# RDG0818/MAZero

Measured on NVIDIA B200. Metric: mcts_sims_per_sec, higher is better.
Workload: dtype bf16

## Files before the change

mazero_b200/csrc/infer_hmma.cuh:

```cuda
#pragma once
#include <cuda_bf16.h>

#include "../../include/maz_infer.h"
#include "umma.cuh"

namespace maz {
namespace hmma {

using namespace umma;

constexpr int H = 128, NHEAD = 8, HD = 16, GH = 64, PH = 32, SUP = 11, NLAYER = 3;
constexpr int NCHUNK = MAZ_INFER_NCHUNK, NSLOT = 3;
constexpr int TM = 32;
#ifndef MAZ_HMMA_NQ
#define MAZ_HMMA_NQ 4
#endif
constexpr int NQ = MAZ_HMMA_NQ;
constexpr int NT = H / NQ / 8;
constexpr int GT = GH / NQ / 8;
constexpr int CW = H / NQ, FW = GH / NQ;
static_assert(NQ == 4 || NQ == 8, "NQ");
constexpr int NCONS = 64 * NQ, NTHREADS = NCONS + 32;
constexpr int PAD = 8;
constexpr int LDA = (H + PAD) * 2;
// ... 117 lines not shown
#pragma unroll GEMM_UNROLL
    for (int ks = 0; ks < KS; ++ks) {
        const int cur = ks & 1, nxt = cur ^ 1;
        if (ks + 1 < KS) {
            ldsm4(aa + 32u * (ks + 1), a[nxt]);
#pragma unroll
            for (int p = 0; p < NT / 2; ++p) ldsm4(wa + (uint32_t)(16 * p) * ldw + 32u * (ks + 1), b[nxt][p]);
        }
#pragma unroll
        for (int p = 0; p < NT / 2; ++p) {
            mma16816(acc[2 * p], a[cur], b[cur][p][0], b[cur][p][1]);
            mma16816(acc[2 * p + 1], a[cur], b[cur][p][2], b[cur][p][3]);
        }
    }
}
template <int NT>
__device__ __forceinline__ void gemm_rt(float (&acc)[NT][4], const Thr &th, uint32_t a_tile, int lda, uint32_t w_slot, int ldw, int n0, int K)
{
    const uint32_t aa = th.a_addr(a_tile, lda), wa = th.w_addr(w_slot, ldw, n0);
#pragma unroll 1
    for (int k0 = 0; k0 < K; k0 += 16) {
        uint32_t a[4], b[NT / 2][4];
        ldsm4(aa + 2u * k0, a);
#pragma unroll
        for (int p = 0; p < NT / 2; ++p) ldsm4(wa + (uint32_t)(16 * p) * ldw + 2u * k0, b[p]);
#pragma unroll
        for (int p = 0; p < NT / 2; ++p) {
            mma16816(acc[2 * p], a, b[p][0], b[p][1]);
            mma16816(acc[2 * p + 1], a, b[p][2], b[p][3]);
        }
    }
}

__device__ __forceinline__ void issue_chunk(const Desc &d, int k, int slot, uint64_t *bar_full)
{
    HSM_DECL;
    const uint32_t nbytes = (d.dbg_flags & 4) ? 16u : d.chunk_bytes[k];
    const uint8_t *src = reinterpret_cast<const uint8_t *>(d.wpk) + d.chunk_off[k];
    uint8_t *dst = hsm + OFF_W + (size_t)slot * SLOT_BYTES;
    mbar_expect_tx(&bar_full[slot], nbytes);
    for (uint32_t o = 0; o < nbytes; o += PIECE) {
        const uint32_t n = (nbytes - o < PIECE) ? (nbytes - o) : PIECE;
        bulk_g2s(dst + o, src + o, n, &bar_full[slot]);
    }
}

struct Ring {
    uint64_t *full, *empty;
    int c;
    __device__ __forceinline__ uint32_t acquire(int ahead = 0)
    {
        const int cc = c + ahead, s = cc % NSLOT;
        mbar_wait(&full[s], (cc / NSLOT) & 1);
        return sbase() + OFF_W + (uint32_t)s * SLOT_BYTES;
    }
    __device__ __forceinline__ void release(int lane, int n = 1)
    {
        __syncwarp();
        if (lane == 0)
            for (int i = 0; i < n; ++i) mbar_arrive(&empty[(c + i) % NSLOT]);
        c += n;
    }
};

__device__ __forceinline__ void cta_sync() { named_bar_sync(1, NCONS); }

template <int NT>
__device__ __forceinline__ void zero(float (&acc)[NT][4])
{
#pragma unroll
    for (int i = 0; i < NT; ++i) acc[i][0] = acc[i][1] = acc[i][2] = acc[i][3] = 0.f;
}
template <int NT>
__device__ __forceinline__ void copy(float (&dst)[NT][4], const float (&src)[NT][4])
{
#pragma unroll
    for (int i = 0; i < NT; ++i) { dst[i][0] = src[i][0]; dst[i][1] = src[i][1]; dst[i][2] = src[i][2]; dst[i][3] = src[i][3]; }
}

template <int NT>
__device__ __forceinline__ void add_bias(float (&acc)[NT][4], const Thr &th, uint32_t b, int n0)
{
#pragma unroll
    for (int nt = 0; nt < NT; ++nt) {
        const float2 v = ldp2(b + 4u * (n0 + 8 * nt + 2 * th.t));
        acc[nt][0] += v.x; acc[nt][1] += v.y; acc[nt][2] += v.x; acc[nt][3] += v.y;
    }
}
template <int NT>
__device__ __forceinline__ void store_tile(uint32_t tile, int ld, const Thr &th, int n0, const float (&acc)[NT][4])
{
#pragma unroll
    for (int nt = 0; nt < NT; ++nt) {
        const int c = n0 + 8 * nt + 2 * th.t;
        sts32(tile + (uint32_t)th.rA * ld + 2u * c, pack2(acc[nt][0], acc[nt][1]));
        sts32(tile + (uint32_t)th.rB * ld + 2u * c, pack2(acc[nt][2], acc[nt][3]));
    }
}
// ... 8 lines not shown
}

template <int NT>
__device__ __forceinline__ void stats_write(const float (&v)[NT][4], const Thr &th, uint32_t stat)
{
    float s0 = 0.f, q0 = 0.f, s1 = 0.f, q1 = 0.f;
#pragma unroll
    for (int nt = 0; nt < NT; ++nt) {
        s0 += v[nt][0] + v[nt][1]; q0 += v[nt][0] * v[nt][0] + v[nt][1] * v[nt][1];
        s1 += v[nt][2] + v[nt][3]; q1 += v[nt][2] * v[nt][2] + v[nt][3] * v[nt][3];
    }
#pragma unroll
    for (int o = 1; o <= 2; o <<= 1) {
        s0 += __shfl_xor_sync(0xffffffffu, s0, o); q0 += __shfl_xor_sync(0xffffffffu, q0, o);
        s1 += __shfl_xor_sync(0xffffffffu, s1, o); q1 += __shfl_xor_sync(0xffffffffu, q1, o);
    }
    if (th.t == 0) {
        sts2f(stat + (uint32_t)(th.rA * NQ + th.nq) * 8u, s0, q0);
        sts2f(stat + (uint32_t)(th.rB * NQ + th.nq) * 8u, s1, q1);
    }
}
__device__ __forceinline__ void stats_read(uint32_t stat, int row, float inv_width, float &mean, float &rstd)
{
    float4 v[NQ / 2];
#pragma unroll
    for (int i = 0; i < NQ / 2; ++i) v[i] = lds4v(stat + (uint32_t)row * (NQ * 8u) + 16u * i);
    float s = 0.f, q = 0.f;
#pragma unroll
    for (int i = 0; i < NQ / 2; ++i) { s += v[i].x + v[i].z; q += v[i].y + v[i].w; }
    mean = s * inv_width;
    rstd = rsqrtf(fmaxf(q * inv_width - mean * mean, 0.f) + 1e-5f);
}

__device__ __forceinline__ void layer_norm128(float (&x)[NT][4], const Thr &th, uint32_t gam, uint32_t bet, int n0, bool relu_after)
{
    const uint32_t stat = sbase() + OFF_STAT;
    stats_write<NT>(x, th, stat);
    cta_sync();
    float mA, sA, mB, sB;
    stats_read(stat, th.rA, 1.f / H, mA, sA);
    stats_read(stat, th.rB, 1.f / H, mB, sB);
#pragma unroll
    for (int nt = 0; nt < NT; ++nt) {
        const int c = n0 + 8 * nt + 2 * th.t;
        const float2 gg = ldp2(gam + 4u * c), bb = ldp2(bet + 4u * c);
        x[nt][0] = (x[nt][0] - mA) * sA * gg.x + bb.x; x[nt][1] = (x[nt][1] - mA) * sA * gg.y + bb.y;
        x[nt][2] = (x[nt][2] - mB) * sB * gg.x + bb.x; x[nt][3] = (x[nt][3] - mB) * sB * gg.y + bb.y;
    }
    if (relu_after) relu<NT>(x);
}

__device__ __forceinline__ RowInfo row_info(int r)
{
    uint32_t a, b, c, e;
    lds4u(sbase() + OFF_ROW + 16u * r, a, b, c, e);
    RowInfo ri;
    ri.root = (int)a; ri.agent = (int)b; ri.valid = (int)c; ri.r0 = (int)e;
    return ri;
}

static __device__ __noinline__ void stage_gather(const Desc &d, const SimIo io)
{
    HSM_DECL;
    const int tid = threadIdx.x, r = tid >> 3, part = tid & 7;
    if (tid >= TM * 8) return;
    const RowInfo ri = row_info(r);
    uint32_t w[8] = {0, 0, 0, 0, 0, 0, 0, 0};
    int action = -1;
    if (ri.valid) {
        const int ix = io.idx_x ? __ldcg(io.idx_x + ri.root) : 0;
        if (d.greedy_pool == nullptr || d.cur < 0)
            action = __ldcg(io.actions + (size_t)ri.root * d.N + ri.agent);
        else if (ri.agent == d.cur)
            action = __ldcg(io.actions + ri.root);
        else if (ri.agent < d.cur)
            action = d.factor ? __ldcg(d.factor + (size_t)ri.root * d.N + ri.agent) : 0;
        else
            action = __ldcg(d.greedy_pool + ((size_t)ix * d.B + ri.root) * d.N + ri.agent);
        const float *h = d.pool + ((size_t)ix * d.B + ri.root) * (size_t)(d.N * H) + (size_t)ri.agent * H + part * 16;
#pragma unroll
        for (int i = 0; i < 4; ++i) {
            const float4 v = __ldcg(reinterpret_cast<const float4 *>(h) + i);
            w[2 * i] = pack2(v.x, v.y);
            w[2 * i + 1] = pack2(v.z, v.w);
        }
    }
    uint4 *dst = reinterpret_cast<uint4 *>(hsm + OFF_HH + (size_t)r * LDA + part * 32);
    dst[0] = make_uint4(w[0], w[1], w[2], w[3]);
    dst[1] = make_uint4(w[4], w[5], w[6], w[7]);
    if (part * 8 < d.KA) {
        const int c0 = part * 8;
        uint32_t o[4];
#pragma unroll
        for (int i = 0; i < 4; ++i) o[i] = pack2((c0 + 2 * i == action) ? 1.f : 0.f, (c0 + 2 * i + 1 == action) ? 1.f : 0.f);
        *reinterpret_cast<uint4 *>(hsm + OFF_ONE + (size_t)r * LDO + c0 * 2) = make_uint4(o[0], o[1], o[2], o[3]);
    }
}

static __device__ __noinline__ void stage_inproj(const Desc &d, Ring &ring, float (&xio)[NT][4])
{
    const Thr th;
    const uint32_t sb = sbase();
    const int n0 = CW * th.nq, ldo = (d.KA + PAD) * 2;
    float x[NT][4];
    zero<NT>(x);
    uint32_t w = ring.acquire();
    gemm_fixed<NT, 8>(x, th, sb + OFF_HH, LDA, w, LDA, n0);
    ring.release(th.lane);
    w = ring.acquire();
    gemm_rt<NT>(x, th, sb + OFF_ONE, LDO, w, ldo, n0, d.KA);
    ring.release(th.lane);
    add_bias<NT>(x, th, sb + OFF_P + 4u * d.o_bin, n0);
    const uint32_t pA = sb + OFF_P + 4u * (d.o_pos + row_info(th.rA).agent * H), pB = sb + OFF_P + 4u * (d.o_pos + row_info(th.rB).agent * H);
#pragma unroll
    for (int nt = 0; nt < NT; ++nt) {
        const int c = n0 + 8 * nt + 2 * th.t;
        const float2 a = ldp2(pA + 4u * c), b = ldp2(pB + 4u * c);
        x[nt][0] = fmaxf(x[nt][0], 0.f) + a.x; x[nt][1] = fmaxf(x[nt][1], 0.f) + a.y;
        x[nt][2] = fmaxf(x[nt][2], 0.f) + b.x; x[nt][3] = fmaxf(x[nt][3], 0.f) + b.y;
    }
    store_tile<NT>(sb + OFF_X, LDA, th, n0, x);
    copy<NT>(xio, x);
    cta_sync();
}

static __device__ __noinline__ void stage_qkv(Ring &ring, uint32_t lv)
{
    const Thr th;
    const uint32_t sb = sbase();
    const int n0 = CW * th.nq;
    float acc[3 * NT][4];
    zero<3 * NT>(acc);
    uint32_t wa[3];
#pragma unroll
    for (int i = 0; i < 3; ++i) wa[i] = th.w_addr(ring.acquire(i), LDA, n0);
    const uint32_t aa = th.a_addr(sb + OFF_X, LDA);
    constexpr int PW = NT / 2, NP = 3 * PW;
    uint32_t a[2][4], b[2][NP][4];
    ldsm4(aa, a[0]);
#pragma unroll
    for (int p = 0; p < NP; ++p) ldsm4(wa[p / PW] + (uint32_t)(16 * (p % PW)) * LDA, b[0][p]);
#pragma unroll GEMM_UNROLL
    for (int ks = 0; ks < 8; ++ks) {
        const int cur = ks & 1, nxt = cur ^ 1;
        if (ks + 1 < 8) {
            ldsm4(aa + 32u * (ks + 1), a[nxt]);
#pragma unroll
            for (int p = 0; p < NP; ++p) ldsm4(wa[p / PW] + (uint32_t)(16 * (p % PW)) * LDA + 32u * (ks + 1), b[nxt][p]);
        }
#pragma unroll
        for (int p = 0; p < NP; ++p) {
            mma16816(acc[2 * p], a[cur], b[cur][p][0], b[cur][p][1]);
            mma16816(acc[2 * p + 1], a[cur], b[cur][p][2], b[cur][p][3]);
        }
    }
    ring.release(th.lane, 3);
#pragma unroll
    for (int which = 0; which < 3; ++which) {
#pragma unroll
        for (int nt = 0; nt < NT; ++nt) {
            const int c = n0 + 8 * nt + 2 * th.t;
            const float2 bv = ldp2(lv + 4u * (which * H + c));
            const float *v = acc[which * NT + nt];
            sts32(sb + OFF_Q + (uint32_t)th.rA * LDQ + 2u * (which * H + c), pack2(v[0] + bv.x, v[1] + bv.y));
            sts32(sb + OFF_Q + (uint32_t)th.rB * LDQ + 2u * (which * H + c), pack2(v[2] + bv.x, v[3] + bv.y));
        }
    }
    cta_sync();
}

__device__ __forceinline__ void unpack16(const uint32_t (&w)[8], float (&f)[16])
{
#pragma unroll
    for (int i = 0; i < 8; ++i) {
        f[2 * i] = __uint_as_float(w[i] << 16);
        f[2 * i + 1] = __uint_as_float(w[i] & 0xffff0000u);
    }
}
__device__ __forceinline__ void lds32B(uint32_t saddr, uint32_t (&w)[8])
{
    lds4u(saddr, w[0], w[1], w[2], w[3]);
    lds4u(saddr + 16u, w[4], w[5], w[6], w[7]);
}

template <int NN>
__device__ __forceinline__ void attention_small(uint32_t qbase, int r0, int hh, const float (&q)[16], float (&o)[16])
{
    float s[NN];
    uint32_t kw[NN][8], vw[NN][8];
#pragma unroll
    for (int j = 0; j < NN; ++j) {
        const uint32_t kr = qbase + (uint32_t)(r0 + j) * LDQ + H * 2 + hh * 32;
        lds32B(kr, kw[j]);
        lds32B(kr + H * 2, vw[j]);
    }
#pragma unroll
    for (int j = 0; j < NN; ++j) {
        float k[16];
        unpack16(kw[j], k);
        float a = 0.f, b = 0.f;
#pragma unroll
        for (int i = 0; i < 16; i += 2) { a += q[i] * k[i]; b += q[i + 1] * k[i + 1]; }
        s[j] = a + b;
    }
    float m = s[0];
#pragma unroll
    for (int j = 1; j < NN; ++j) m = fmaxf(m, s[j]);
    float l = 0.f;
#pragma unroll
    for (int j = 0; j < NN; ++j) { s[j] = __expf(s[j] - m); l += s[j]; }
    const float inv = 1.f / l;
#pragma unroll
    for (int i = 0; i < 16; ++i) o[i] = 0.f;
#pragma unroll
    for (int j = 0; j < NN; ++j) {
        float v[16];
        unpack16(vw[j], v);
        const float p = s[j] * inv;
#pragma unroll
        for (int i = 0; i < 16; ++i) o[i] += p * v[i];
    }
}

static __device__ __noinline__ void stage_attention(const Desc &d)
{
    const uint32_t sb = sbase(), qbase = sb + OFF_Q;
    const int tid = threadIdx.x, r = tid >> 3, hh = tid & 7;
    if (tid >= TM * NHEAD) {
        cta_sync();
        return;
    }
    const RowInfo ri = row_info(r);
    const int N = d.N;
    float q[16], o[16];
    {
        uint32_t w[8];
        lds32B(qbase + (uint32_t)r * LDQ + hh * 32, w);
        unpack16(w, q);
#pragma unroll
        for (int i = 0; i < 16; ++i) q[i] *= 0.25f;
    }
    if (N <= 4) {
        switch (N) {
            case 1: attention_small<1>(qbase, ri.r0, hh, q, o); break;
            case 2: attention_small<2>(qbase, ri.r0, hh, q, o); break;
            case 3: attention_small<3>(qbase, ri.r0, hh, q, o); break;
            default: attention_small<4>(qbase, ri.r0, hh, q, o); break;
        }
    } else {
#pragma unroll
        for (int i = 0; i < 16; ++i) o[i] = 0.f;
        float m = -INFINITY, lsum = 0.f;
#pragma unroll 1
        for (int j = 0; j < N; ++j) {
            const uint32_t kr = qbase + (uint32_t)(ri.r0 + j) * LDQ + H * 2 + hh * 32;
            uint32_t kw[8], vw[8];
            lds32B(kr, kw);
            lds32B(kr + H * 2, vw);
            float k[16], v[16];
            unpack16(kw, k);
            unpack16(vw, v);
            float s = 0.f;
#pragma unroll
            for (int i = 0; i < 16; ++i) s += q[i] * k[i];
            const float mn = fmaxf(m, s);
            const float corr = __expf(m - mn), p = __expf(s - mn);
            lsum = lsum * corr + p;
#pragma unroll
            for (int i = 0; i < 16; ++i) o[i] = o[i] * corr + p * v[i];
            m = mn;
        }
        const float inv = 1.f / lsum;
#pragma unroll
        for (int i = 0; i < 16; ++i) o[i] *= inv;
    }
    uint4 a, b;
    a.x = pack2(o[0], o[1]); a.y = pack2(o[2], o[3]); a.z = pack2(o[4], o[5]); a.w = pack2(o[6], o[7]);
    b.x = pack2(o[8], o[9]); b.y = pack2(o[10], o[11]); b.z = pack2(o[12], o[13]); b.w = pack2(o[14], o[15]);
    sts4(sb + OFF_T + (uint32_t)r * LDA + hh * 32, a);
    sts4(sb + OFF_T + (uint32_t)r * LDA + hh * 32 + 16, b);
    cta_sync();
}

static __device__ __noinline__ void stage_residual_ln(Ring &ring, float (&xio)[NT][4], uint32_t bias, uint32_t gam, uint32_t bet)
{
    const Thr th;
    const uint32_t sb = sbase();
    const int n0 = CW * th.nq;
    float x[NT][4];
    copy<NT>(x, xio);
    const uint32_t w = ring.acquire();
    gemm_fixed<NT, 8>(x, th, sb + OFF_T, LDA, w, LDA, n0);
    ring.release(th.lane);
    add_bias<NT>(x, th, bias, n0);
    layer_norm128(x, th, gam, bet, n0, false);
    store_tile<NT>(sb + OFF_X, LDA, th, n0, x);
    copy<NT>(xio, x);
    cta_sync();
}

static __device__ __noinline__ void stage_linear_relu(Ring &ring, uint32_t bias)
{
    const Thr th;
    const uint32_t sb = sbase();
    const int n0 = CW * th.nq;
    float acc[NT][4];
    zero<NT>(acc);
    const uint32_t w = ring.acquire();
    gemm_fixed<NT, 8>(acc, th, sb + OFF_X, LDA, w, LDA, n0);
    ring.release(th.lane);
    add_bias<NT>(acc, th, bias, n0);
    relu<NT>(acc);
    store_tile<NT>(sb + OFF_T, LDA, th, n0, acc);
    cta_sync();
}

static __device__ __noinline__ void stage_dynamics(const Desc &d, Ring &ring, const SimIo io)
{
    const Thr th;
    const uint32_t sb = sbase();
    const int n0 = CW * th.nq, ldo = (d.KA + PAD) * 2;
    const uint32_t dv = sb + OFF_P + 4u * d.o_dyn;
    float acc[NT][4];
    zero<NT>(acc);
    uint32_t w = ring.acquire();
    gemm_fixed<NT, 8>(acc, th, sb + OFF_HH, LDA, w, LDA, n0);
    ring.release(th.lane);
    w = ring.acquire();
    gemm_rt<NT>(acc, th, sb + OFF_ONE, LDO, w, ldo, n0, d.KA);
    ring.release(th.lane);
    w = ring.acquire();
    gemm_fixed<NT, 8>(acc, th, sb + OFF_X, LDA, w, LDA, n0);
    ring.release(th.lane);
    add_bias<NT>(acc, th, dv, n0);
    layer_norm128(acc, th, dv + 4u * 128, dv + 4u * 256, n0, true);
    store_tile<NT>(sb + OFF_T, LDA, th, n0, acc);
    cta_sync();
    zero<NT>(acc);
    w = ring.acquire();
    gemm_fixed<NT, 8>(acc, th, sb + OFF_T, LDA, w, LDA, n0);
    ring.release(th.lane);
    add_bias<NT>(acc, th, dv + 4u * 384, n0);
    layer_norm128(acc, th, dv + 4u * 512, dv + 4u * 640, n0, true);
    store_tile<NT>(sb + OFF_X, LDA, th, n0, acc);
    cta_sync();
    const RowInfo ra = row_info(th.rA), rb = row_info(th.rB);
    float2 hv[2][NT];
#pragma unroll
    for (int hf = 0; hf < 2; ++hf) {
        const RowInfo &ri = hf ? rb : ra;
        const int ix = (ri.valid && io.idx_x) ? io.idx_x[ri.root - io.root0] : 0;
        const float *hp = d.pool + ((size_t)ix * d.B + (ri.valid ? ri.root : 0)) * (size_t)(d.N * H) + (size_t)ri.agent * H;
#pragma unroll
        for (int nt = 0; nt < NT; ++nt)
            hv[hf][nt] = ri.valid ? __ldcg(reinterpret_cast<const float2 *>(hp + n0 + 8 * nt + 2 * th.t)) : make_float2(0.f, 0.f);
    }
    zero<NT>(acc);
    w = ring.acquire();
    gemm_fixed<NT, 8>(acc, th, sb + OFF_X, LDA, w, LDA, n0);
    ring.release(th.lane);
    add_bias<NT>(acc, th, dv + 4u * 768, n0);
#pragma unroll
    for (int hf = 0; hf < 2; ++hf) {
        const RowInfo &ri = hf ? rb : ra;
        float *nh = io.next_hidden + (size_t)(ri.valid ? ri.root : 0) * (d.N * H) + (size_t)ri.agent * H;
#pragma unroll
        for (int nt = 0; nt < NT; ++nt) {
            acc[nt][2 * hf] += hv[hf][nt].x;
            acc[nt][2 * hf + 1] += hv[hf][nt].y;
            if (ri.valid) *reinterpret_cast<float2 *>(nh + n0 + 8 * nt + 2 * th.t) = make_float2(acc[nt][2 * hf], acc[nt][2 * hf + 1]);
        }
    }
    store_tile<NT>(sb + OFF_T, LDA, th, n0, acc);
    cta_sync();
}

__device__ __forceinline__ void gnn_phase_a(const float (&acc)[NT][4], const Thr &th, uint32_t G, uint32_t b)
{
    const int f0 = FW * th.nq + 2 * th.t;
#pragma unroll
    for (int tl = 0; tl < GT; ++tl) {
        const float2 bg = ldp2(b + 4u * (f0 + 8 * tl));
        sts2f(G + 4u * (th.rA * LDG + f0 + 8 * tl), acc[tl][0] + bg.x, acc[tl][1] + bg.y);
        sts2f(G + 4u * (th.rB * LDG + f0 + 8 * tl), acc[tl][2] + bg.x, acc[tl][3] + bg.y);
    }
}
template <int NN>
__device__ __forceinline__ void agent_sums(uint32_t G, int f0, int r0A, int r0B, float2 (&sa)[GT], float2 (&sc)[GT])
{
    float2 a[NN][GT], c[NN][GT];
#pragma unroll
    for (int j = 0; j < NN; ++j)
#pragma unroll
        for (int tl = 0; tl < GT; ++tl) {
            a[j][tl] = lds2f(G + 4u * ((r0A + j) * LDG + f0 + 8 * tl));
            c[j][tl] = lds2f(G + 4u * ((r0B + j) * LDG + f0 + 8 * tl));
        }
#pragma unroll
    for (int j = 0; j < NN; ++j)
#pragma unroll
        for (int tl = 0; tl < GT; ++tl) {
            sa[tl].x += a[j][tl].x; sa[tl].y += a[j][tl].y; sc[tl].x += c[j][tl].x; sc[tl].y += c[j][tl].y;
        }
}
__device__ __forceinline__ void gnn_phase_b(const float (&acc)[NT][4], const Thr &th, uint32_t G, uint32_t b, uint32_t stat, int N, int r0A,
                                            int r0B, float (&y)[GT][4])
{
    const int f0 = FW * th.nq + 2 * th.t;
    float2 sa[GT], sc[GT];
#pragma unroll
    for (int tl = 0; tl < GT; ++tl) sa[tl] = sc[tl] = make_float2(0.f, 0.f);
    {
        int j = 0;
#pragma unroll 1
        for (; j + 3 <= N; j += 3) agent_sums<3>(G, f0, r0A + j, r0B + j, sa, sc);
#pragma unroll 1
        for (; j < N; ++j) agent_sums<1>(G, f0, r0A + j, r0B + j, sa, sc);
    }
#pragma unroll
    for (int tl = 0; tl < GT; ++tl) {
        const float2 bn = ldp2(b + 4u * (GH + f0 + 8 * tl));
        y[tl][0] = fmaxf(sa[tl].x + acc[GT + tl][0] + bn.x, 0.f); y[tl][1] = fmaxf(sa[tl].y + acc[GT + tl][1] + bn.y, 0.f);
        y[tl][2] = fmaxf(sc[tl].x + acc[GT + tl][2] + bn.x, 0.f); y[tl][3] = fmaxf(sc[tl].y + acc[GT + tl][3] + bn.y, 0.f);
    }
    stats_write<GT>(y, th, stat);
}
__device__ __forceinline__ void gnn_phase_c(const Thr &th, uint32_t stat, float (&y)[GT][4])
{
    float mA, sA, mB, sB;
    stats_read(stat, th.rA, 1.f / GH, mA, sA);
    stats_read(stat, th.rB, 1.f / GH, mB, sB);
#pragma unroll
    for (int tl = 0; tl < GT; ++tl) {
        y[tl][0] = (y[tl][0] - mA) * sA; y[tl][1] = (y[tl][1] - mA) * sA;
        y[tl][2] = (y[tl][2] - mB) * sB; y[tl][3] = (y[tl][3] - mB) * sB;
    }
}

static __device__ __noinline__ void stage_heads1(const Desc &d, Ring &ring)
{
    const Thr th;
    const uint32_t sb = sbase();
    const int n0 = CW * th.nq, ldo = (d.KA + PAD) * 2;
    float aR[NT][4], aV[NT][4], aP[2][4];
    zero<NT>(aR); zero<NT>(aV); zero<2>(aP);
    uint32_t w = ring.acquire();
    gemm_fixed<NT, 8>(aR, th, sb + OFF_T, LDA, w, LDA, n0);
    ring.release(th.lane);
    w = ring.acquire();
    gemm_rt<NT>(aR, th, sb + OFF_ONE, LDO, w, ldo, n0, d.KA);
    ring.release(th.lane);
    w = ring.acquire();
    gemm_fixed<NT, 8>(aV, th, sb + OFF_T, LDA, w, LDA, n0);
    ring.release(th.lane);
    w = ring.acquire();
    if (th.nq < 2) gemm_fixed<2, 8>(aP, th, sb + OFF_T, LDA, w, LDA, 16 * th.nq);
    ring.release(th.lane);
    const uint32_t G = sb + OFF_Q, stat = sb + OFF_STAT, pr = sb + OFF_P + 4u * d.o_rg, pvv = sb + OFF_P + 4u * d.o_vg;
    const uint32_t pp = sb + OFF_P + 4u * d.o_pol;
    gnn_phase_a(aR, th, G + 4u * G_R, pr);
    gnn_phase_a(aV, th, G + 4u * G_V, pvv);
    if (th.nq < 2) add_bias<2>(aP, th, pp, 16 * th.nq);
    stats_write<2>(aP, th, stat + 2 * STAT_SET);
    cta_sync();
    const int r0A = row_info(th.rA).r0, r0B = row_info(th.rB).r0;
    float yR[GT][4], yV[GT][4];
    gnn_phase_b(aR, th, G + 4u * G_R, pr, stat, d.N, r0A, r0B, yR);
    gnn_phase_b(aV, th, G + 4u * G_V, pvv, stat + STAT_SET, d.N, r0A, r0B, yV);
    if (th.nq < 2) {
        float mA, sA, mB, sB;
        stats_read(stat + 2 * STAT_SET, th.rA, 1.f / PH, mA, sA);
        stats_read(stat + 2 * STAT_SET, th.rB, 1.f / PH, mB, sB);
#pragma unroll
        for (int tl = 0; tl < 2; ++tl) {
            const int c = 16 * th.nq + 8 * tl + 2 * th.t;
            const float2 gg = ldp2(pp + 4u * (PH + c)), bb = ldp2(pp + 4u * (2 * PH + c));
            const float v0 = fmaxf((aP[tl][0] - mA) * sA * gg.x + bb.x, 0.f), v1 = fmaxf((aP[tl][1] - mA) * sA * gg.y + bb.y, 0.f);
            const float v2 = fmaxf((aP[tl][2] - mB) * sB * gg.x + bb.x, 0.f), v3 = fmaxf((aP[tl][3] - mB) * sB * gg.y + bb.y, 0.f);
            sts32(sb + OFF_PH + (uint32_t)th.rA * LDP + 2u * c, pack2(v0, v1));
            sts32(sb + OFF_PH + (uint32_t)th.rB * LDP + 2u * c, pack2(v2, v3));
        }
    }
    cta_sync();
    gnn_phase_c(th, stat, yR);
    gnn_phase_c(th, stat + STAT_SET, yV);
    store_tile<GT>(sb + OFF_X, LDA, th, FW * th.nq, yR);
    store_tile<GT>(sb + OFF_X, LDA, th, GH + FW * th.nq, yV);
    cta_sync();
}

__device__ __forceinline__ float support_to_scalar(const float (&v)[SUP])
{
    float m = v[0];
#pragma unroll
    for (int k = 1; k < SUP; ++k) m = fmaxf(m, v[k]);
    float s = 0.f, x = 0.f;
#pragma unroll
    for (int k = 0; k < SUP; ++k) {
        const float e = __expf(v[k] - m);
        s += e;
        x += e * (float)(k - 5);
    }
    x /= s;
    const float eps = 0.001f;
    const float r = (sqrtf(1.f + 4.f * eps * (fabsf(x) + 1.f + eps)) - 1.f) / (2.f * eps);
    float out = r * r - 1.f;
    out = (x < 0.f) ? -out : out;
    if (!(out == out)) out = 0.f;
    if (fabsf(out) < eps) out = 0.f;
    return out;
}

static __device__ __noinline__ void stage_heads2(const Desc &d, Ring &ring, const SimIo io, long long *hs_clk)
{
    const Thr th;
    const uint32_t sb = sbase();
    const int n0 = CW * th.nq, ldg = (GH + PAD) * 2;
    const int N = d.N, A = d.A, tid = threadIdx.x;
    int hs_n = 40;
#define HS() \
    if (hs_clk && hs_n < 64) hs_clk[hs_n++] = clock64();
    HS();
    float aR[NT][4], aV[NT][4], aP[2][4];
    zero<NT>(aR); zero<NT>(aV); zero<2>(aP);
    uint32_t w = ring.acquire();
    gemm_fixed<NT, 4>(aR, th, sb + OFF_X, LDA, w, ldg, n0);
    ring.release(th.lane);
    w = ring.acquire();
    gemm_fixed<NT, 4>(aV, th, sb + OFF_X + GH * 2, LDA, w, ldg, n0);
    ring.release(th.lane);
    w = ring.acquire();
    const int pc0 = 16 * th.nq;
    if (pc0 < d.NAP) gemm_fixed<2, 2>(aP, th, sb + OFF_PH, LDP, w, LDP, pc0);
    ring.release(th.lane);
    const uint32_t G = sb + OFF_Q, stat = sb + OFF_STAT, pr = sb + OFF_P + 4u * (d.o_rg + 128), pvv = sb + OFF_P + 4u * (d.o_vg + 128);
    const uint32_t PL = G + 4u * PL0;
    HS();
    gnn_phase_a(aR, th, G + 4u * G_R, pr);
    gnn_phase_a(aV, th, G + 4u * G_V, pvv);
    if (pc0 < d.NAP) {
        const uint32_t b2 = sb + OFF_P + 4u * (d.o_pol + 96);
#pragma unroll
        for (int tl = 0; tl < 2; ++tl) {
            const int c = pc0 + 8 * tl + 2 * th.t;
            const float2 bb = ldp2(b2 + 4u * c);
            sts2f(PL + 4u * (th.rA * 48 + c), aP[tl][0] + bb.x, aP[tl][1] + bb.y);
            sts2f(PL + 4u * (th.rB * 48 + c), aP[tl][2] + bb.x, aP[tl][3] + bb.y);
        }
    }
    cta_sync();
    HS();
    const int r0A = row_info(th.rA).r0, r0B = row_info(th.rB).r0;
    float yR[GT][4], yV[GT][4];
    gnn_phase_b(aR, th, G + 4u * G_R, pr, stat, N, r0A, r0B, yR);
    gnn_phase_b(aV, th, G + 4u * G_V, pvv, stat + STAT_SET, N, r0A, r0B, yV);
    const uint32_t YB = sb + OFF_X;
#pragma unroll
    for (int tl = 0; tl < GT; ++tl) {
        const int f = FW * th.nq + 8 * tl + 2 * th.t;
        sts2f(YB + 4u * (Y_R + th.rA * GH + f), yR[tl][0], yR[tl][1]);
        sts2f(YB + 4u * (Y_R + th.rB * GH + f), yR[tl][2], yR[tl][3]);
        sts2f(YB + 4u * (Y_V + th.rA * GH + f), yV[tl][0], yV[tl][1]);
        sts2f(YB + 4u * (Y_V + th.rB * GH + f), yV[tl][2], yV[tl][3]);
    }
// ... 125 lines not shown
        const int rpt = tile_rpt(d), rl = tid / N, agent = tid - rl * N;
        const int root = blockIdx.x * rpt + rl;
        RowInfo ri;
        ri.valid = (rl < rpt) && (root < d.B);
        ri.root = root; ri.agent = (rl < rpt) ? agent : 0;
        ri.r0 = (rl < rpt) ? rl * N : 0;
        reinterpret_cast<RowInfo *>(hsm + OFF_ROW)[tid] = ri;
    }
}

__device__ __forceinline__ void produce_weights(const Desc &d, uint64_t *bar_full, uint64_t *bar_empty, uint64_t *bar_vec, int rounds)
{
    HSM_DECL;
    mbar_expect_tx(bar_vec, (uint32_t)d.vec_floats * 4u);
    bulk_g2s(hsm + OFF_P, d.vec, (uint32_t)d.vec_floats * 4u, bar_vec);
    const int total = rounds * NCHUNK;
#pragma unroll 1
    for (int c = 0, k = 0; c < total; ++c, k = (k + 1 == NCHUNK) ? 0 : k + 1) {
        const int s = c % NSLOT;
        if (c >= NSLOT) mbar_wait_backoff(&bar_empty[s], ((c / NSLOT) - 1) & 1);
        issue_chunk(d, k, s, bar_full);
    }
}

__device__ __forceinline__ void setup_head_copies(const Desc &d)
{
    const uint32_t sb = sbase();
    for (int i = threadIdx.x; i < 2 * SUP * GH; i += NCONS) {
        const int f = i % GH, rest = i / GH, k = rest % SUP, kind = rest / SUP;
        sts1f(sb + OFF_VP + 4u * ((kind * SUP + k) * LDV + f), lds1v(sb + OFF_P + 4u * ((kind ? d.o_vg : d.o_rg) + 256 + k * GH + f)));
    }
}

__device__ __forceinline__ void infer_stages(const Desc &d, const SimIo io, Ring &ring, long long *clk)
{
    int ts_n = 2;
#define TS() \
    if (clk && ts_n < 64) clk[ts_n++] = clock64();
    TS();
    float x[NT][4];
    stage_inproj(d, ring, x);
    TS();
    const uint32_t pbase = sbase() + OFF_P;
#pragma unroll 1
    for (int l = 0; l < NLAYER; ++l) {
        const uint32_t lv = pbase + 4u * (d.o_layer + l * 1280);
        stage_qkv(ring, lv);
        TS();
        stage_attention(d);
        TS();
        stage_residual_ln(ring, x, lv + 4u * 384, lv + 4u * 512, lv + 4u * 640);
        TS();
        stage_linear_relu(ring, lv + 4u * 768);
        TS();
        stage_residual_ln(ring, x, lv + 4u * 896, lv + 4u * 1024, lv + 4u * 1152);
        TS();
    }
    TS();
    stage_dynamics(d, ring, io);
    TS();
    stage_heads1(d, ring);
    TS();
    stage_heads2(d, ring, io, clk);
    TS();
#undef TS
}

#ifndef MAZ_HMMA_NO_KERNEL
__global__ void __launch_bounds__(NTHREADS, 1) k_recurrent_inference_small(const __grid_constant__ Desc d)
{
    HSM_DECL;
    __shared__ __align__(8) uint64_t bar_full[NSLOT], bar_empty[NSLOT], bar_vec;
    const int tid = threadIdx.x, warp = tid >> 5;

    if (tid == 0) {
        for (int i = 0; i < NSLOT; ++i) { mbar_init(&bar_full[i], 1); mbar_init(&bar_empty[i], NCONS / 32); }
        mbar_init(&bar_vec, 1);
        mbar_fence_init();
    }
    setup_rows(d);
    __syncthreads();

    if (warp == NCONS / 32) {
        if ((tid & 31) == 0) produce_weights(d, bar_full, bar_empty, &bar_vec, 1);
        return;
    }
    Ring ring{bar_full, bar_empty, 0};
    long long *clk = (d.dbg_clock != nullptr && blockIdx.x == 0 && tid == 0) ? d.dbg_clock : nullptr;
    if (clk) clk[0] = clock64();
    asm volatile("griddepcontrol.wait;" ::: "memory");
    asm volatile("griddepcontrol.launch_dependents;" ::: "memory");
    const SimIo io = io_from_desc(d);
    stage_gather(d, io);
    if (clk) clk[1] = clock64();
    mbar_wait(&bar_vec, 0);
    setup_head_copies(d);
    cta_sync();
    infer_stages(d, io, ring, clk);
}
#endif

}
}
```

mazero_b200/csrc/search_persist.cuh:

```cuda
#pragma once
#include "infer_hmma.cuh"
#include "tree_step.cuh"

namespace maz {
namespace persist {

using namespace hmma;

struct SearchParams {
    Desc d;
    TreeLayout L;
    char *arena;
    const float *lam_pow, *logterm;
    const double *sqrtn;
    int table_len;
    float discount;
    int K, S;
    int *g_err;
    int *idx_y;
    int *greedy_w;
    float *rec_r, *rec_v, *rec_p, *rec_b;
    int *rec_ix, *rec_act;
    long long *tree_clock;
};
// ... 158 lines not shown
                    if (lane == 0) { P.rec_r[o] = x_r[warp]; P.rec_v[o] = x_v[warp]; }
                    for (int t = lane; t < (int)NA; t += 32) {
                        P.rec_p[o * NA + t] = x_p[(size_t)warp * NA + t];
                        P.rec_b[o * NA + t] = x_b[(size_t)warp * NA + t];
                    }
                }
                expand_backup_device<false>(L, tb, hdr, hot, P.lam_pow, s, P.discount, P.K, x_r + warp, x_v + warp, x_p + (size_t)warp * NA,
                                            x_b + (size_t)warp * NA, scr, lane, P.g_err, kProf ? tree : -1);
            }
            __syncwarp();
            if (kProf && s > 0 && L.dbg_clock != nullptr && tree == 0 && lane == 0) {
                const int order[11] = {0, 1, 2, 11, 12, 13, 14, 15, 3, 4, 5};
                for (int i = 1; i < 11; ++i) L.dbg_clock[16 + i] += L.dbg_clock[order[i]] - L.dbg_clock[order[i - 1]];
            }
            const long long q1 = tree_clk ? clock64() : 0;
            if (s < P.S) {
                select_next_device(L, tb, hdr, hot, P.logterm, P.sqrtn, P.table_len, P.discount, warp, lane, &scr, x_i, nullptr, x_a,
                                   P.g_err);
                __syncwarp();
                const int ix = x_i[warp];
                if (P.rec_ix != nullptr) {
                    const size_t o = (size_t)s * B + tree;
                    if (lane == 0) P.rec_ix[o] = ix;
                    for (int j = lane; j < L.N; j += 32) P.rec_act[o * L.N + j] = x_a[warp * L.N + j];
                }
                gather_root(d, tree, warp, ix, x_a + warp * L.N, lane);
            }
            if (tree_clk) {
                const long long q2 = clock64();
                const int pl = hdr->path_len;
                tc_eb += q1 - q0; tc_sel += q2 - q1; tc_len += pl; tc_max = pl > tc_max ? pl : tc_max;
            }
        }
        cta_sync();
        const long long t2 = cta_clk ? clock64() : 0;
        if (cta_clk) {
            sum_tree += t2 - t1;
            if (clk && s > 0) clk[2 * (s - 1) + 1] = t2 - t1;
        }
        if (s == P.S) break;
        io.next_hidden = d.next_hidden + (size_t)s * B * (size_t)(d.N * H);
        io.greedy = P.greedy_w ? P.greedy_w + (size_t)(s + 1) * B * d.N : nullptr;
        long long *sclk = (clk && s == P.S / 2) ? P.tree_clock + 2 * P.S + 4 * (long long)gridDim.x : nullptr;
        if (sclk) { sclk[0] = t2; sclk[1] = t2; }
        infer_stages(d, io, ring, sclk);
        cta_sync();
        if (cta_clk) {
            const long long t3 = clock64();
            sum_inf += t3 - t2;
            if (clk) clk[2 * s] = t3 - t2;
        }
    }
    if (has_tree && lane < 16) reinterpret_cast<int *>(f_hdr(tb))[lane] = reinterpret_cast<const int *>(hdr)[lane];
    if (tree_clk) { tree_clk[0] = tc_eb; tree_clk[1] = tc_sel; tree_clk[2] = tc_len; tree_clk[3] = tc_max; }
    if (cta_clk) {
        cta_clk[0] = clock64() - k0;
        cta_clk[1] = (long long)(globaltimer_ns() - g0);
        cta_clk[2] = sum_inf;
        cta_clk[3] = sum_tree;
    }
}

}
}
```

profiles/prof_search.py:

```python
import os
import sys

import numpy as np
import torch

sys.path.insert(0, os.path.dirname(os.path.dirname(os.path.abspath(__file__))))
from mazero_b200.inference import SmacInference
from mazero_b200.mcts_sampled import SampledMCTS, _DevicePlan, clear_caches
from mazero_b200.synthetic import WORKLOADS, NetworkOutput, SearchConfig, random_state_dict, root_hidden


def main():
    wl = sys.argv[1] if len(sys.argv) > 1 else "3m"
    reps = int(sys.argv[2]) if len(sys.argv) > 2 else 10
    strategies = sys.argv[3:] or ["persistent", "graph"]
    N, A, B, S, K = WORKLOADS[wl]
    B = int(os.environ.get("MAZ_B", B))
    cur = os.environ.get("MAZ_CUR")
    cur = None if cur is None else int(cur)
    dev = torch.device("cuda:0")
    inf = SmacInference(random_state_dict(N, A, seed=0, head_scale=30.0), N, A, device=dev, mode="bf16")
    cfg = SearchConfig(A, S, K)
    flush = torch.empty(256 << 20, dtype=torch.uint8, device=dev)
    for strat in strategies:
# ... 27 lines not shown
        call = clk.cpu().numpy()
        c = call[:2 * S].reshape(S, 2)
        per = call[2 * S:2 * S + 4 * ncta].reshape(-1, 4)
        per = per[per[:, 0] > 0]
        if plan.native is not None and plan.native.strategy == "persistent":
            assert plan.native.roots_per_cta() == rpc, (plan.native.roots_per_cta(), rpc)
        pt = call[2 * S + 4 * ncta + 64:][:4 * B].reshape(B, 4) if len(per) else np.zeros((0, 4))
        if len(pt) and pt[:, 0].any():
            order = np.argsort(-(pt[:, 0] + pt[:, 1]))
            print(f"  per tree (cycles/sim): expand+backup mean {pt[:, 0].mean() / S:.0f} max {pt[:, 0].max() / S:.0f}; select mean "
                  f"{pt[:, 1].mean() / S:.0f} max {pt[:, 1].max() / S:.0f}; mean depth {pt[:, 2].mean() / S:.2f}, max depth {pt[:, 3].max()}")
            print("  slowest trees [expand+backup/sim, select/sim, mean depth, max depth]: " +
                  "; ".join(f"{pt[i, 0] / S:.0f} {pt[i, 1] / S:.0f} {pt[i, 2] / S:.1f} {pt[i, 3]}" for i in order[:6]))
            d = pt[:, 2] / S
            for lo, hi in ((0, 2), (2, 3), (3, 5), (5, 8), (8, 100)):
                m = (d >= lo) & (d < hi)
                if m.any():
                    print(f"    mean depth in [{lo},{hi}): {m.sum()} trees, expand+backup {pt[m, 0].mean() / S:.0f}, select {pt[m, 1].mean() / S:.0f} cycles/sim")
        ts = call[2 * S + 4 * ncta + 64 + 4 * B:][:32]
        if ts[:6].all():
            nm = {0: "start", 1: "header", 2: "prefetch issued", 11: "beta/probs staged", 12: "cdf", 13: "sampled", 14: "keys merged",
                  15: "children", 3: "expansion done", 4: "backup", 5: "minmax+header"}
            order = [0, 1, 2, 11, 12, 13, 14, 15, 3, 4, 5]
            print("  tree 0, phase cycles per simulation (mean over the search): " +
                  ", ".join(f"{nm[b]} {ts[16 + i + 1] / S:.0f}" for i, b in enumerate(order[1:])))
        st_all = call[2 * S + 4 * ncta:][:64]
        hs = st_all[40:]
        hs = hs[hs > 0]
        if len(hs) > 2:
            print("  heads2 phases (cycles): " + " ".join(str(int(v)) for v in np.diff(hs)))
        st = st_all[:40]
        st = st[st > 0]
        if len(st) > 2:
            names = ["gather", "sync", "inproj"] + [f"L{l}.{x}" for l in range(3) for x in ("qkv", "attn", "out+ln", "lin1", "lin2+ln")] + \
                    ["-", "dynamics", "heads1", "heads2"]
            dl = np.diff(st)
            print("  stage cycles (CTA 0, middle simulation): " + ", ".join(f"{n} {int(v)}" for n, v in zip(names, dl)))
        if len(per):
            ghz = per[:, 0] / np.maximum(per[:, 1], 1)
            print(f"  {len(per)} CTAs: total cycles mean {per[:, 0].mean():.0f} min {per[:, 0].min()} max {per[:, 0].max()}; "
                  f"ns mean {per[:, 1].mean():.0f} max {per[:, 1].max()}; SM clock {ghz.mean():.3f} GHz; "
                  f"inference cycles/sim mean {per[:, 2].mean() / S:.0f} max {per[:, 2].max() / S:.0f}; "
                  f"tree cycles/sim mean {per[:, 3].mean() / S:.0f} min {per[:, 3].min() / S:.0f} max {per[:, 3].max() / S:.0f}")
        print(f"{wl} B={B} cur={cur} strategy={strat} ({plan.native.strategy if plan.native else 'legacy'}): "
              f"{t.mean():.3f} ms/search (min {t.min():.3f} max {t.max():.3f}) -> {B * S / t.mean() / 1e3:.2f} M root-sims/s"
              + (f"; CTA0 cycles/sim: inference {c[:, 0].mean():.0f} tree {c[:, 1].mean():.0f}" if c.any() else ""))
        out = {k: v.clone() for k, v in plan.turn_out[0].items()}
        plan.close()
        del plan
    clear_caches()


if __name__ == "__main__":
    main()
```

Baseline: 18.20 million.

## Prefetch weight fragments into registers before barriers and use half-CTA syncs

Adds a templated pre-load path for the persistent search kernel. Each GEMM stage loads its weight B-fragments from the ring slot into registers and releases the slot before the CTA barrier, so the barrier wait overlaps the weight fetch. Trailing full-CTA barriers are removed, and several are replaced by per-row-half named barriers, so only warps sharing rows wait on each other. The tree-phase barrier is folded into the first inference stage. The cost is higher register pressure from holding whole weight-fragment sets, and more reliance on subtle barrier ordering for correctness.

```diff
diff --git a/mazero_b200/csrc/infer_hmma.cuh b/mazero_b200/csrc/infer_hmma.cuh
--- a/mazero_b200/csrc/infer_hmma.cuh
+++ b/mazero_b200/csrc/infer_hmma.cuh
@@ -173,6 +173,37 @@
     }
 }
 
+template <int NT, int KS>
+struct BFrag {
+    uint32_t b[KS][NT / 2][4];
+};
+template <int NT, int KS>
+__device__ __forceinline__ void load_b(BFrag<NT, KS> &f, const Thr &th, uint32_t w_slot, int ldw, int n0)
+{
+    const uint32_t wa = th.w_addr(w_slot, ldw, n0);
+#pragma unroll
+    for (int ks = 0; ks < KS; ++ks)
+#pragma unroll
+        for (int p = 0; p < NT / 2; ++p) ldsm4(wa + (uint32_t)(16 * p) * ldw + 32u * ks, f.b[ks][p]);
+}
+template <int NT, int KS>
+__device__ __forceinline__ void gemm_b(float (&acc)[NT][4], const Thr &th, uint32_t a_tile, int lda, const BFrag<NT, KS> &f)
+{
+    const uint32_t aa = th.a_addr(a_tile, lda);
+    uint32_t a[2][4];
+    ldsm4(aa, a[0]);
+#pragma unroll
+    for (int ks = 0; ks < KS; ++ks) {
+        const int cur = ks & 1;
+        if (ks + 1 < KS) ldsm4(aa + 32u * (ks + 1), a[cur ^ 1]);
+#pragma unroll
+        for (int p = 0; p < NT / 2; ++p) {
+            mma16816(acc[2 * p], a[cur], f.b[ks][p][0], f.b[ks][p][1]);
+            mma16816(acc[2 * p + 1], a[cur], f.b[ks][p][2], f.b[ks][p][3]);
+        }
+    }
+}
+
 __device__ __forceinline__ void issue_chunk(const Desc &d, int k, int slot, uint64_t *bar_full)
 {
     HSM_DECL;
@@ -205,6 +236,14 @@
 };
 
 __device__ __forceinline__ void cta_sync() { named_bar_sync(1, NCONS); }
+__device__ __forceinline__ void half_sync(int mt) { named_bar_sync(2 + mt, NCONS / 2); }
+
+template <int NT, int KS>
+__device__ __forceinline__ void take_b(BFrag<NT, KS> &f, Ring &ring, const Thr &th, int ldw, int n0)
+{
+    load_b<NT, KS>(f, th, ring.acquire(), ldw, n0);
+    ring.release(th.lane);
+}
 
 template <int NT>
 __device__ __forceinline__ void zero(float (&acc)[NT][4])
@@ -279,11 +318,13 @@
     rstd = rsqrtf(fmaxf(q * inv_width - mean * mean, 0.f) + 1e-5f);
 }
 
-__device__ __forceinline__ void layer_norm128(float (&x)[NT][4], const Thr &th, uint32_t gam, uint32_t bet, int n0, bool relu_after)
+__device__ __forceinline__ void layer_norm128(float (&x)[NT][4], const Thr &th, uint32_t gam, uint32_t bet, int n0, bool relu_after,
+                                              bool half = false)
 {
     const uint32_t stat = sbase() + OFF_STAT;
     stats_write<NT>(x, th, stat);
-    cta_sync();
+    if (half) half_sync(th.mt);
+    else cta_sync();
     float mA, sA, mB, sB;
     stats_read(stat, th.rA, 1.f / H, mA, sA);
     stats_read(stat, th.rB, 1.f / H, mB, sB);
@@ -344,17 +385,27 @@
     }
 }
 
-static __device__ __noinline__ void stage_inproj(const Desc &d, Ring &ring, float (&xio)[NT][4])
+
+template <bool kPre>
+static __device__ __noinline__ void stage_inproj(const Desc &d, Ring &ring, float (&xio)[NT][4], long long *t_sync)
 {
     const Thr th;
     const uint32_t sb = sbase();
     const int n0 = CW * th.nq, ldo = (d.KA + PAD) * 2;
     float x[NT][4];
     zero<NT>(x);
+    if constexpr (kPre) {
+        BFrag<NT, 8> f;
+        take_b(f, ring, th, LDA, n0);
+        cta_sync();
+        if (t_sync) *t_sync = clock64();
+        gemm_b(x, th, sb + OFF_HH, LDA, f);
+    } else {
+        const uint32_t w = ring.acquire();
+        gemm_fixed<NT, 8>(x, th, sb + OFF_HH, LDA, w, LDA, n0);
+        ring.release(th.lane);
+    }
     uint32_t w = ring.acquire();
-    gemm_fixed<NT, 8>(x, th, sb + OFF_HH, LDA, w, LDA, n0);
-    ring.release(th.lane);
-    w = ring.acquire();
     gemm_rt<NT>(x, th, sb + OFF_ONE, LDO, w, ldo, n0, d.KA);
     ring.release(th.lane);
     add_bias<NT>(x, th, sb + OFF_P + 4u * d.o_bin, n0);
@@ -368,9 +419,10 @@
     }
     store_tile<NT>(sb + OFF_X, LDA, th, n0, x);
     copy<NT>(xio, x);
-    cta_sync();
-}
-
+    if (!kPre) cta_sync();
+}
+
+template <bool kPre>
 static __device__ __noinline__ void stage_qkv(Ring &ring, uint32_t lv)
 {
     const Thr th;
@@ -378,6 +430,7 @@
     const int n0 = CW * th.nq;
     float acc[3 * NT][4];
     zero<3 * NT>(acc);
+    if (kPre) half_sync(th.mt);
     uint32_t wa[3];
 #pragma unroll
     for (int i = 0; i < 3; ++i) wa[i] = th.w_addr(ring.acquire(i), LDA, n0);
@@ -413,7 +466,7 @@
             sts32(sb + OFF_Q + (uint32_t)th.rB * LDQ + 2u * (which * H + c), pack2(v[2] + bv.x, v[3] + bv.y));
         }
     }
-    cta_sync();
+    if (!kPre) cta_sync();
 }
 
 __device__ __forceinline__ void unpack16(const uint32_t (&w)[8], float (&f)[16])
@@ -469,12 +522,14 @@
     }
 }
 
+template <bool kPre>
 static __device__ __noinline__ void stage_attention(const Desc &d)
 {
     const uint32_t sb = sbase(), qbase = sb + OFF_Q;
     const int tid = threadIdx.x, r = tid >> 3, hh = tid & 7;
+    if (kPre) cta_sync();
     if (tid >= TM * NHEAD) {
-        cta_sync();
+        if (!kPre) cta_sync();
         return;
     }
     const RowInfo ri = row_info(r);
@@ -526,26 +581,43 @@
     b.x = pack2(o[8], o[9]); b.y = pack2(o[10], o[11]); b.z = pack2(o[12], o[13]); b.w = pack2(o[14], o[15]);
     sts4(sb + OFF_T + (uint32_t)r * LDA + hh * 32, a);
     sts4(sb + OFF_T + (uint32_t)r * LDA + hh * 32 + 16, b);
-    cta_sync();
-}
-
-static __device__ __noinline__ void stage_residual_ln(Ring &ring, float (&xio)[NT][4], uint32_t bias, uint32_t gam, uint32_t bet)
+    if (!kPre) cta_sync();
+}
+
+template <bool kPre>
+__device__ __forceinline__ void gemm_chunk(float (&acc)[NT][4], Ring &ring, const Thr &th, uint32_t tile, int n0, bool half = false)
+{
+    if constexpr (kPre) {
+        BFrag<NT, 8> f;
+        take_b(f, ring, th, LDA, n0);
+        if (half) half_sync(th.mt);
+        else cta_sync();
+        gemm_b(acc, th, tile, LDA, f);
+    } else {
+        const uint32_t w = ring.acquire();
+        gemm_fixed<NT, 8>(acc, th, tile, LDA, w, LDA, n0);
+        ring.release(th.lane);
+    }
+}
+
+template <bool kPre>
+static __device__ __noinline__ void stage_residual_ln(Ring &ring, float (&xio)[NT][4], uint32_t bias, uint32_t gam, uint32_t bet,
+                                                      bool half_open)
 {
     const Thr th;
     const uint32_t sb = sbase();
     const int n0 = CW * th.nq;
     float x[NT][4];
     copy<NT>(x, xio);
-    const uint32_t w = ring.acquire();
-    gemm_fixed<NT, 8>(x, th, sb + OFF_T, LDA, w, LDA, n0);
-    ring.release(th.lane);
+    gemm_chunk<kPre>(x, ring, th, sb + OFF_T, n0, half_open);
     add_bias<NT>(x, th, bias, n0);
-    layer_norm128(x, th, gam, bet, n0, false);
+    layer_norm128(x, th, gam, bet, n0, false, kPre);
     store_tile<NT>(sb + OFF_X, LDA, th, n0, x);
     copy<NT>(xio, x);
-    cta_sync();
-}
-
+    if (!kPre) cta_sync();
+}
+
+template <bool kPre>
 static __device__ __noinline__ void stage_linear_relu(Ring &ring, uint32_t bias)
 {
     const Thr th;
@@ -553,15 +625,14 @@
     const int n0 = CW * th.nq;
     float acc[NT][4];
     zero<NT>(acc);
-    const uint32_t w = ring.acquire();
-    gemm_fixed<NT, 8>(acc, th, sb + OFF_X, LDA, w, LDA, n0);
-    ring.release(th.lane);
+    gemm_chunk<kPre>(acc, ring, th, sb + OFF_X, n0, true);
     add_bias<NT>(acc, th, bias, n0);
     relu<NT>(acc);
     store_tile<NT>(sb + OFF_T, LDA, th, n0, acc);
-    cta_sync();
-}
-
+    if (!kPre) cta_sync();
+}
+
+template <bool kPre>
 static __device__ __noinline__ void stage_dynamics(const Desc &d, Ring &ring, const SimIo io)
 {
     const Thr th;
@@ -576,21 +647,17 @@
     w = ring.acquire();
     gemm_rt<NT>(acc, th, sb + OFF_ONE, LDO, w, ldo, n0, d.KA);
     ring.release(th.lane);
-    w = ring.acquire();
-    gemm_fixed<NT, 8>(acc, th, sb + OFF_X, LDA, w, LDA, n0);
-    ring.release(th.lane);
+    gemm_chunk<kPre>(acc, ring, th, sb + OFF_X, n0, true);
     add_bias<NT>(acc, th, dv, n0);
-    layer_norm128(acc, th, dv + 4u * 128, dv + 4u * 256, n0, true);
+    layer_norm128(acc, th, dv + 4u * 128, dv + 4u * 256, n0, true, kPre);
     store_tile<NT>(sb + OFF_T, LDA, th, n0, acc);
-    cta_sync();
+    if (!kPre) cta_sync();
     zero<NT>(acc);
-    w = ring.acquire();
-    gemm_fixed<NT, 8>(acc, th, sb + OFF_T, LDA, w, LDA, n0);
-    ring.release(th.lane);
+    gemm_chunk<kPre>(acc, ring, th, sb + OFF_T, n0, true);
     add_bias<NT>(acc, th, dv + 4u * 384, n0);
-    layer_norm128(acc, th, dv + 4u * 512, dv + 4u * 640, n0, true);
+    layer_norm128(acc, th, dv + 4u * 512, dv + 4u * 640, n0, true, kPre);
     store_tile<NT>(sb + OFF_X, LDA, th, n0, acc);
-    cta_sync();
+    if (!kPre) cta_sync();
     const RowInfo ra = row_info(th.rA), rb = row_info(th.rB);
     float2 hv[2][NT];
 #pragma unroll
@@ -603,9 +670,7 @@
             hv[hf][nt] = ri.valid ? __ldcg(reinterpret_cast<const float2 *>(hp + n0 + 8 * nt + 2 * th.t)) : make_float2(0.f, 0.f);
     }
     zero<NT>(acc);
-    w = ring.acquire();
-    gemm_fixed<NT, 8>(acc, th, sb + OFF_X, LDA, w, LDA, n0);
-    ring.release(th.lane);
+    gemm_chunk<kPre>(acc, ring, th, sb + OFF_X, n0, true);
     add_bias<NT>(acc, th, dv + 4u * 768, n0);
 #pragma unroll
     for (int hf = 0; hf < 2; ++hf) {
@@ -619,7 +684,7 @@
         }
     }
     store_tile<NT>(sb + OFF_T, LDA, th, n0, acc);
-    cta_sync();
+    if (!kPre) cta_sync();
 }
 
 __device__ __forceinline__ void gnn_phase_a(const float (&acc)[NT][4], const Thr &th, uint32_t G, uint32_t b)
@@ -684,6 +749,7 @@
     }
 }
 
+template <bool kPre>
 static __device__ __noinline__ void stage_heads1(const Desc &d, Ring &ring)
 {
     const Thr th;
@@ -691,10 +757,8 @@
     const int n0 = CW * th.nq, ldo = (d.KA + PAD) * 2;
     float aR[NT][4], aV[NT][4], aP[2][4];
     zero<NT>(aR); zero<NT>(aV); zero<2>(aP);
+    gemm_chunk<kPre>(aR, ring, th, sb + OFF_T, n0, true);
     uint32_t w = ring.acquire();
-    gemm_fixed<NT, 8>(aR, th, sb + OFF_T, LDA, w, LDA, n0);
-    ring.release(th.lane);
-    w = ring.acquire();
     gemm_rt<NT>(aR, th, sb + OFF_ONE, LDO, w, ldo, n0, d.KA);
     ring.release(th.lane);
     w = ring.acquire();
@@ -733,7 +797,7 @@
     gnn_phase_c(th, stat + STAT_SET, yV);
     store_tile<GT>(sb + OFF_X, LDA, th, FW * th.nq, yR);
     store_tile<GT>(sb + OFF_X, LDA, th, GH + FW * th.nq, yV);
-    cta_sync();
+    if (!kPre) cta_sync();
 }
 
 __device__ __forceinline__ float support_to_scalar(const float (&v)[SUP])
@@ -758,6 +822,7 @@
     return out;
 }
 
+template <bool kPre>
 static __device__ __noinline__ void stage_heads2(const Desc &d, Ring &ring, const SimIo io, long long *hs_clk)
 {
     const Thr th;
@@ -770,13 +835,23 @@
     HS();
     float aR[NT][4], aV[NT][4], aP[2][4];
     zero<NT>(aR); zero<NT>(aV); zero<2>(aP);
-    uint32_t w = ring.acquire();
-    gemm_fixed<NT, 4>(aR, th, sb + OFF_X, LDA, w, ldg, n0);
-    ring.release(th.lane);
-    w = ring.acquire();
-    gemm_fixed<NT, 4>(aV, th, sb + OFF_X + GH * 2, LDA, w, ldg, n0);
-    ring.release(th.lane);
-    w = ring.acquire();
+    if constexpr (kPre) {
+        BFrag<NT, 4> fr, fv;
+        load_b<NT, 4>(fr, th, ring.acquire(0), ldg, n0);
+        load_b<NT, 4>(fv, th, ring.acquire(1), ldg, n0);
+        ring.release(th.lane, 2);
+        cta_sync();
+        gemm_b(aR, th, sb + OFF_X, LDA, fr);
+        gemm_b(aV, th, sb + OFF_X + GH * 2, LDA, fv);
+    } else {
+        uint32_t w = ring.acquire();
+        gemm_fixed<NT, 4>(aR, th, sb + OFF_X, LDA, w, ldg, n0);
+        ring.release(th.lane);
+        w = ring.acquire();
+        gemm_fixed<NT, 4>(aV, th, sb + OFF_X + GH * 2, LDA, w, ldg, n0);
+        ring.release(th.lane);
+    }
+    const uint32_t w = ring.acquire();
     const int pc0 = 16 * th.nq;
     if (pc0 < d.NAP) gemm_fixed<2, 2>(aP, th, sb + OFF_PH, LDP, w, LDP, pc0);
     ring.release(th.lane);
@@ -968,36 +1043,37 @@
     }
 }
 
-__device__ __forceinline__ void infer_stages(const Desc &d, const SimIo io, Ring &ring, long long *clk)
+template <bool kPre>
+__device__ __forceinline__ void infer_stages(const Desc &d, const SimIo io, Ring &ring, long long *clk, long long *t_sync = nullptr)
 {
     int ts_n = 2;
 #define TS() \
     if (clk && ts_n < 64) clk[ts_n++] = clock64();
     TS();
     float x[NT][4];
-    stage_inproj(d, ring, x);
+    stage_inproj<kPre>(d, ring, x, t_sync);
     TS();
     const uint32_t pbase = sbase() + OFF_P;
 #pragma unroll 1
     for (int l = 0; l < NLAYER; ++l) {
         const uint32_t lv = pbase + 4u * (d.o_layer + l * 1280);
-        stage_qkv(ring, lv);
+        stage_qkv<kPre>(ring, lv);
         TS();
-        stage_attention(d);
+        stage_attention<kPre>(d);
         TS();
-        stage_residual_ln(ring, x, lv + 4u * 384, lv + 4u * 512, lv + 4u * 640);
+        stage_residual_ln<kPre>(ring, x, lv + 4u * 384, lv + 4u * 512, lv + 4u * 640, false);
         TS();
-        stage_linear_relu(ring, lv + 4u * 768);
+        stage_linear_relu<kPre>(ring, lv + 4u * 768);
         TS();
-        stage_residual_ln(ring, x, lv + 4u * 896, lv + 4u * 1024, lv + 4u * 1152);
+        stage_residual_ln<kPre>(ring, x, lv + 4u * 896, lv + 4u * 1024, lv + 4u * 1152, true);
         TS();
     }
     TS();
-    stage_dynamics(d, ring, io);
+    stage_dynamics<kPre>(d, ring, io);
     TS();
-    stage_heads1(d, ring);
+    stage_heads1<kPre>(d, ring);
     TS();
-    stage_heads2(d, ring, io, clk);
+    stage_heads2<kPre>(d, ring, io, clk);
     TS();
 #undef TS
 }
@@ -1032,7 +1108,7 @@
     mbar_wait(&bar_vec, 0);
     setup_head_copies(d);
     cta_sync();
-    infer_stages(d, io, ring, clk);
+    infer_stages<false>(d, io, ring, clk);
 }
 #endif
 
diff --git a/mazero_b200/csrc/search_persist.cuh b/mazero_b200/csrc/search_persist.cuh
--- a/mazero_b200/csrc/search_persist.cuh
+++ b/mazero_b200/csrc/search_persist.cuh
@@ -214,23 +214,32 @@
                 tc_eb += q1 - q0; tc_sel += q2 - q1; tc_len += pl; tc_max = pl > tc_max ? pl : tc_max;
             }
         }
-        cta_sync();
-        const long long t2 = cta_clk ? clock64() : 0;
-        if (cta_clk) {
-            sum_tree += t2 - t1;
-            if (clk && s > 0) clk[2 * (s - 1) + 1] = t2 - t1;
-        }
-        if (s == P.S) break;
+        long long t2 = 0;
+        if (s == P.S) {
+            if (kProf) {
+                cta_sync();
+                if (cta_clk) {
+                    t2 = clock64();
+                    sum_tree += t2 - t1;
+                    if (clk) clk[2 * (s - 1) + 1] = t2 - t1;
+                }
+            }
+            break;
+        }
         io.next_hidden = d.next_hidden + (size_t)s * B * (size_t)(d.N * H);
         io.greedy = P.greedy_w ? P.greedy_w + (size_t)(s + 1) * B * d.N : nullptr;
         long long *sclk = (clk && s == P.S / 2) ? P.tree_clock + 2 * P.S + 4 * (long long)gridDim.x : nullptr;
-        if (sclk) { sclk[0] = t2; sclk[1] = t2; }
-        infer_stages(d, io, ring, sclk);
+        if (sclk) { sclk[0] = t1; sclk[1] = clock64(); }
+        infer_stages<true>(d, io, ring, sclk, cta_clk ? &t2 : nullptr);
         cta_sync();
         if (cta_clk) {
             const long long t3 = clock64();
+            sum_tree += t2 - t1;
             sum_inf += t3 - t2;
-            if (clk) clk[2 * s] = t3 - t2;
+            if (clk) {
+                if (s > 0) clk[2 * (s - 1) + 1] = t2 - t1;
+                clk[2 * s] = t3 - t2;
+            }
         }
     }
     if (has_tree && lane < 16) reinterpret_cast<int *>(f_hdr(tb))[lane] = reinterpret_cast<const int *>(hdr)[lane];
diff --git a/profiles/prof_search.py b/profiles/prof_search.py
--- a/profiles/prof_search.py
+++ b/profiles/prof_search.py
@@ -83,7 +83,7 @@
         st = st_all[:40]
         st = st[st > 0]
         if len(st) > 2:
-            names = ["gather", "sync", "inproj"] + [f"L{l}.{x}" for l in range(3) for x in ("qkv", "attn", "out+ln", "lin1", "lin2+ln")] + \
+            names = ["tree step (warp 0)", "-", "inproj"] +[f"L{l}.{x}" for l in range(3) for x in ("qkv", "attn", "out+ln", "lin1", "lin2+ln")] + \
                     ["-", "dynamics", "heads1", "heads2"]
             dl = np.diff(st)
             print("  stage cycles (CTA 0, middle simulation): " + ", ".join(f"{n} {int(v)}" for n, v in zip(names, dl)))
```

New measurement: 18.62 million (median of 6 runs). +2.3%, better.
